# nichmorgan/better-search-rag-rust

Hardware: AMD Instinct MI355X
Metric: queries/sec + p50 latency, 768-d top-10 over N vectors @1/2/4/8 GPU (higher is better)
Workload: dtype f32; 1 GPU; configs[2]: 10M x 768 f32 corpus sharded over the N GPUs, 1000 batched queries, top-10; rows_total=10000000, rows_per_gpu_rank0=10000000, queries=1000, top_k=10, dim=768, parallelism=corpus sharded over 1 GPU(s) (interval_by_rank)

## Files before the change

better-search-rag-rust_amd/csrc/k_filter.hip:

```cpp
#include <cstdlib>
#include "bsr_device.hpp"
#include "kernels.hpp"

#include <hip/hip_ext.h>

#include <limits.h>
#include <math.h>

#include <algorithm>
#include <type_traits>
#include <utility>

namespace bsr {

typedef __attribute__((ext_vector_type(4))) int i32x4_t;
typedef __attribute__((ext_vector_type(16))) int i32x16_t;
typedef __attribute__((address_space(3))) void lds_void_t;

constexpr int kSlots = 4;
constexpr int kSliceB = 64;
constexpr int kWCap = 256;
constexpr int kThreads = 512;

__device__ __forceinline__ void wait_vm0() { asm volatile("s_waitcnt vmcnt(0)" ::: "memory"); }
// ... 307 lines not shown
        BSR_QS_N(1) BSR_QS_N(2) BSR_QS_N(3) BSR_QS_N(4) BSR_QS_N(5) BSR_QS_N(6) BSR_QS_N(7) BSR_QS_N(8)
        BSR_QS_N(9) BSR_QS_N(10) BSR_QS_N(11) BSR_QS_N(12) BSR_QS_N(13) BSR_QS_N(14) BSR_QS_N(15)
        default: qs_wait<0>(); break;
    }
#undef BSR_QS_N
}

#ifdef BSR_FILTER_STAMPS
__device__ __forceinline__ void qs_vm_n(int n) {
#define BSR_QS_V(N) \
    case N: asm volatile("s_waitcnt vmcnt(" #N ")" ::: "memory"); break;
    switch (n) {
        BSR_QS_V(1) BSR_QS_V(2) BSR_QS_V(3) BSR_QS_V(4) BSR_QS_V(5) BSR_QS_V(6) BSR_QS_V(7) BSR_QS_V(8)
        default: asm volatile("s_waitcnt vmcnt(0)" ::: "memory"); break;
    }
#undef BSR_QS_V
}
#endif
typedef __attribute__((ext_vector_type(4))) int i32x4v_t;

template <class F, int... I>
__device__ __forceinline__ void static_for(std::integer_sequence<int, I...>, F&& f) {
    (f(std::integral_constant<int, I>{}), ...);
}

constexpr int kSampleTilesPerWG = 8;

__device__ __forceinline__ uint32_t qs16_swz(uint32_t row) { return ((row >> 3) & 1u) * 2u; }

#ifdef BSR_FILTER_COUNTERS
__device__ unsigned long long g_filter_counters[8];
extern "C" int bsr_lab_filter_counters(unsigned long long* out, int reset) {
    hipError_t e = hipMemcpyFromSymbol(out, HIP_SYMBOL(g_filter_counters), sizeof(g_filter_counters));
    if (e == hipSuccess && reset) {
        static const unsigned long long z[8] = {};
        e = hipMemcpyToSymbol(HIP_SYMBOL(g_filter_counters), z, sizeof(z));
    }
    return (int)e;
}
__device__ unsigned long long g_filter_wg_stamps[4096 * 9];
__device__ uint32_t g_lab_xcd_xor;
extern "C" int bsr_lab_set_xcd_xor(uint32_t v) {
    return (int)hipMemcpyToSymbol(HIP_SYMBOL(g_lab_xcd_xor), &v, sizeof v);
}
__device__ unsigned int g_filter_wg_tiles[4096 * 2];
extern "C" int bsr_lab_filter_wg_tiles(unsigned int* out) {
    return (int)hipMemcpyFromSymbol(out, HIP_SYMBOL(g_filter_wg_tiles), sizeof(g_filter_wg_tiles));
}
extern "C" int bsr_lab_filter_wg_stamps(unsigned long long* out) {
    return (int)hipMemcpyFromSymbol(out, HIP_SYMBOL(g_filter_wg_stamps), sizeof(g_filter_wg_stamps));
}
#define BSR_FCNT(I_) ++fcnt[I_]
#else
#define BSR_FCNT(I_) \
    do {             \
    } while (0)
#endif
#ifdef BSR_FILTER_STAMPS
__device__ unsigned long long g_filter_stamps[8];
extern "C" int bsr_lab_filter_stamps(unsigned long long* out, int reset) {
    hipError_t e = hipMemcpyFromSymbol(out, HIP_SYMBOL(g_filter_stamps), sizeof(g_filter_stamps));
    if (e == hipSuccess && reset) {
        static const unsigned long long z[8] = {};
        e = hipMemcpyToSymbol(HIP_SYMBOL(g_filter_stamps), z, sizeof(z));
    }
    return (int)e;
}
#define BSR_FST(V_)                                                                     \
    do {                                                                                \
        __builtin_amdgcn_sched_barrier(0);                                              \
        asm volatile("s_memtime %0\n\ts_waitcnt lgkmcnt(0)" : "=s"(V_)::"memory");       \
        __builtin_amdgcn_sched_barrier(0);                                              \
    } while (0)
#endif
template <bool EMIT, int NK, bool GANGS = true>
__global__ __launch_bounds__(512, 1) void k_filter_qs16(GemmArgs p) {
    constexpr int GANG = GANGS ? 2 : 0;
    constexpr bool L2 = !GANGS, FW = GANGS;
    constexpr int S = 8, A = 6;
    constexpr int kWaitN = A - 4, kYoung = A - 4, kClaimUse = ((A - 4) % 2 == 0 ? A - 3 : A - 2) + 1;
    constexpr int BM = 128, BN = kFilterTile, NT = 512, SLOT = BM * kSliceB;
    constexpr int CAP = 10;
    static_assert(NK % 2 == 0 && NK >= 2 && NK <= 12, "even slice counts up to 768 bytes");
    constexpr int EM_BYTES = EMIT ? NT * 2 * CAP * 8 : 0;
    constexpr int SB_BYTES = EMIT ? 0 : kSampleTilesPerWG * 4 * BN * 4;
    __shared__ __attribute__((aligned(1024))) uint8_t lds[S * SLOT + EM_BYTES + SB_BYTES + 16];
    float* const sbuf = reinterpret_cast<float*>(lds + S * SLOT + EM_BYTES);
    uint32_t* const lds_ids = reinterpret_cast<uint32_t*>(lds + S * SLOT + EM_BYTES + SB_BYTES);
    const int tid = threadIdx.x, lane = tid & 63, w = tid >> 6;
    const uint32_t wu = __builtin_amdgcn_readfirstlane(tid >> 6);
    uint64_t* const lkeys = reinterpret_cast<uint64_t*>(lds + S * SLOT) + tid;
    uint32_t ecnt[2] = {0, 0};

    const uint32_t b = blockIdx.x, xcd = b & 7, slot = b >> 3;
    const uint32_t G = (gridDim.x >> 3) / p.n_qt;
    const uint32_t n_phys = (p.n_rows + BM - 1) / BM;
    const uint32_t n_rt = !p.s_tiles ? n_phys : EMIT ? n_phys - p.s_tiles : p.s_tiles;
    auto phys = [&](uint32_t lt) -> uint32_t {
        if (!p.s_tiles) return lt;
        return EMIT ? lt + lt / (kSampleTileEvery - 1) : lt * kSampleTileEvery + kSampleTilePhase;
    };
    const bool active = slot < G * p.n_qt;
    const uint32_t qt = active ? slot % p.n_qt : 0;
#ifdef BSR_FILTER_COUNTERS
    const uint32_t g0 = (xcd ^ g_lab_xcd_xor) * G + (active ? slot / p.n_qt : 0);
#else
    const uint32_t g0 = xcd * G + (active ? slot / p.n_qt : 0);
#endif
    const uint32_t RG = 8 * G;
    const uint32_t my_rt = (active && g0 < n_rt) ? (n_rt - 1 - g0) / RG + 1 : 0;
    const uint32_t J = my_rt * NK;
    constexpr uint32_t kEnd = 0xFFFFFFFFu;
    constexpr bool kStaticSched = NK > A;
    const bool dyn = EMIT && kStaticSched && p.tail != nullptr && active;
    const uint32_t n_st = dyn ? n_rt - n_rt / kTailDiv : n_rt;
    const uint32_t my_static = (active && g0 < n_st) ? (n_st - 1 - g0) / RG + 1 : 0;
    const uint32_t n_tail = n_rt - n_st, pool_sz = (n_tail + 7) / 8;
    uint32_t cpool = xcd, pools_tried = 1;
    auto pool_n = [&](uint32_t x) -> uint32_t {
        const uint32_t lo = x * pool_sz;
        return lo >= n_tail ? 0u : min(pool_sz, n_tail - lo);
    };
    auto claim_raw = [&]() -> uint32_t {
        uint32_t z;
        asm volatile("v_mov_b32 %0, 0" : "=v"(z));
        return atomicAdd(p.tail + cpool * p.n_qt + qt + z, 1u);
    };
    auto tail_id = [&](uint32_t v) -> uint32_t {
        for (;;) {
            if (v < pool_n(cpool)) return n_st + cpool * pool_sz + v;
            if (pools_tried == 8) return kEnd;
            ++pools_tried;
            cpool = (cpool + 1) & 7;
            v = atomicAdd(p.tail + cpool * p.n_qt + qt, 1u);
        }
    };
    auto claim = [&]() -> uint32_t { return tail_id(claim_raw()); };
    const bool gang = GANG && EMIT && kStaticSched && active && p.tail != nullptr && p.n_qt >= 2 && p.n_qt <= 4 &&
                      my_static >= kGangMinTiles;
    unsigned long long* const gprog =
        reinterpret_cast<unsigned long long*>(p.tail + 8 * kTailCounters) + (gang ? g0 : 0u);
    auto gang_raw = [&]() -> unsigned long long {
        uint32_t z;
        asm volatile("v_mov_b32 %0, 0" : "=v"(z));
        return atomicAdd(gprog + z, 1ull << (16 * qt));
    };
    auto gang_throttle = [&](unsigned long long old) {
        const uint32_t me = (uint32_t)(old >> (16 * qt)) & 0xFFFFu;
        int lag = 0;
        for (uint32_t j = 0; j < p.n_qt; ++j)
            if (j != qt) lag = max(lag, (int)(int16_t)(uint16_t)(me - ((uint32_t)(old >> (16 * j)) & 0xFFFFu)));
        for (int i = GANG; i < lag && i < GANG + 4; ++i) __builtin_amdgcn_s_sleep(32);
    };

    uint32_t qq[2];
    i32x4v_t fb[2][NK];
    float tau[2], sbq[2];
#pragma unroll
    for (int nb = 0; nb < 2; ++nb) {
        qq[nb] = qt * BN + w * 32 + nb * 16 + (lane & 15);
        const uint8_t* src = p.B + (uint64_t)qq[nb] * p.row_bytes + 16 * (lane >> 4);
#pragma unroll
        for (int kt = 0; kt < NK; ++kt) fb[nb][kt] = *reinterpret_cast<const i32x4v_t*>(src + 64 * kt);
        tau[nb] = EMIT ? p.tau[qq[nb]] : 0.0f;
        sbq[nb] = p.b_scale[qq[nb]];
    }
    auto flush_ring = [&](int nb) {
        const uint32_t nn = ecnt[nb];
        if (nn) {
            const uint32_t gp = atomicAdd(p.cnt + qq[nb], nn);
            for (uint32_t i = 0; i < nn; ++i)
                if (gp + i < p.cap) p.cand[(uint64_t)qq[nb] * p.cap + gp + i] = lkeys[(nb * CAP + i) * NT];
        }
        ecnt[nb] = 0;
        if constexpr (FW) __builtin_amdgcn_s_waitcnt(0x0F70);
    };

    const uint32_t lrow = w * 16 + (lane >> 2);
    const uint32_t lchunk = ((lane & 3) ^ qs16_swz(lrow)) * 16;
    auto tile_src_rt = [&](uint32_t lt, __amdgpu_buffer_rsrc_t& rs, uint32_t& off) {
        const uint32_t rt = phys(lt);
        rs = __builtin_amdgcn_make_buffer_rsrc((void*)(p.A + (uint64_t)rt * BM * p.a_stride), 0,
                                               BM * (uint32_t)p.a_stride, 0x00020000);
        const uint32_t r = (EMIT || rt * BM + lrow < p.n_rows) ? lrow : p.n_rows - 1 - rt * BM;
        off = r * (uint32_t)p.a_stride + lchunk;
    };
    auto tile_src = [&](uint32_t ti, __amdgpu_buffer_rsrc_t& rs, uint32_t& off) { tile_src_rt(g0 + ti * RG, rs, off); };
    constexpr bool kStatic = kStaticSched;
    __amdgpu_buffer_rsrc_t rs_cur, rs_nxt;
    uint32_t off_cur = 0, off_nxt = 0;
    auto dma_static = [&](uint32_t jj, int kt) {
        uint8_t* la = lds + (jj % S) * SLOT + wu * 1024;
        if (kt + A < NK)
            __builtin_amdgcn_raw_ptr_buffer_load_lds(rs_cur, (lds_void_t*)la, 16, off_cur, (kt + A) * kSliceB, 0, 0);
        else
            __builtin_amdgcn_raw_ptr_buffer_load_lds(rs_nxt, (lds_void_t*)la, 16, off_nxt, (kt + A - NK) * kSliceB, 0, 0);
    };
    uint32_t iss_ti = 0, iss_kt = 0, aoff_dma = 0;
    __amdgpu_buffer_rsrc_t rsrc_a;
    auto issue_dma = [&](uint32_t jj) {
        uint8_t* la = lds + (jj % S) * SLOT + wu * 1024;
        __builtin_amdgcn_raw_ptr_buffer_load_lds(rsrc_a, (lds_void_t*)la, 16, aoff_dma, iss_kt * kSliceB, 0, 0);
        if (++iss_kt == NK) {
            iss_kt = 0;
            ++iss_ti;
            if (iss_ti < my_rt) tile_src(iss_ti, rsrc_a, aoff_dma);
        }
    };
    const uint32_t aoff0 = (lane & 15) * kSliceB + (((lane >> 4) ^ qs16_swz(lane & 15)) * 16);
    i32x4v_t fa[4];
    auto read_frag = [&](uint32_t jj, int rb) {
        fa[rb & 3] = *reinterpret_cast<const i32x4v_t*>(lds + (jj % S) * SLOT + rb * 1024 + aoff0);
    };

    i32x4v_t acc[8][2];
    uint32_t cur_id = my_rt ? g0 : kEnd, nxt_id = my_rt > 1 ? g0 + RG : kEnd;
    if (dyn && my_static < 2) {
        if (tid == 0) {
            const uint32_t a0 = my_static ? g0 : claim();
            lds_ids[2] = a0;
            lds_ids[3] = a0 == kEnd ? kEnd : claim();
        }
        __syncthreads();
        cur_id = __builtin_amdgcn_readfirstlane(lds_ids[2]);
        nxt_id = __builtin_amdgcn_readfirstlane(lds_ids[3]);
    } else if (dyn) {
        cur_id = g0;
        nxt_id = g0 + RG;
    }
    const bool any_tile = cur_id != kEnd;
    const uint32_t pre = (dyn ? any_tile : J != 0) ? (uint32_t)A : 0u;
    if (any_tile) {
        tile_src_rt(cur_id, rsrc_a, aoff_dma);
        rs_cur = rsrc_a;
        off_cur = aoff_dma;
        tile_src_rt(nxt_id != kEnd ? nxt_id : cur_id, rs_nxt, off_nxt);
    }
    if (kStatic) {
        for (uint32_t jj = 0; jj < pre; ++jj) {
            uint8_t* la = lds + (jj % S) * SLOT + wu * 1024;
            __builtin_amdgcn_raw_ptr_buffer_load_lds(rs_cur, (lds_void_t*)la, 16, off_cur, jj * kSliceB, 0, 0);
        }
    } else {
        for (uint32_t jj = 0; jj < pre; ++jj) issue_dma(jj);
    }
    qs_barrier(pre >= 3 ? pre - 3 : 0);
    if (any_tile)
#pragma unroll
        for (int rb = 0; rb < 4; ++rb) read_frag(0, rb);

#ifdef BSR_FILTER_COUNTERS
    unsigned long long fcnt[5] = {0, 0, 0, 0, 0};
    if (EMIT && tid == 0 && blockIdx.x < 4096) g_filter_wg_stamps[blockIdx.x * 9] = __builtin_amdgcn_s_memrealtime();
#endif
#ifdef BSR_FILTER_STAMPS
    unsigned long long fst[8] = {0, 0, 0, 0, 0, 0, 0, 0}, st_a, st_b, st_loop0;
    BSR_FST(st_loop0);
#endif
// ... 52 lines not shown
                if (bar_slice ? rb == 6 : rb == 1) {
                    if (kStatic) dma_static(jj + A, kt);
                    else issue_dma(jj + A);
                }
                if (bar_slice && rb == 5 && (kStatic || jj + 1 < J)) {
#ifdef BSR_FILTER_STAMPS
                    if (EMIT) {
                        BSR_FST(st_a);
                        qs_vm_n(kWaitN + ((EMIT && kt <= kYoung) ? 1 + w0_req : 0));
                        BSR_FST(st_b);
                        fst[6] += st_b - st_a;
                        st_a = st_b;
                        asm volatile("s_barrier" ::: "memory");
                        BSR_FST(st_b);
                        fst[kt == 1 ? 3 : 4] += st_b - st_a;
                    } else
#endif
                    qs_wait_n(kWaitN + ((EMIT && kt <= kYoung) ? 1 + w0_req : 0));
                }
                __builtin_amdgcn_sched_barrier(0);
            }
        });
        const float sc[4] = {scv.x, scv.y, scv.z, scv.w};
        bool stored = false;
        if constexpr (!EMIT) {
            if (p.s_compact) {
                const bool part = p.s_tiles && rt * BM + BM > p.n_rows;
#pragma unroll
                for (int g = 0; g < 4; ++g)
#pragma unroll
                    for (int nb = 0; nb < 2; ++nb) {
                        i32x4v_t x = acc[2 * g][nb], y = acc[2 * g + 1][nb];
                        if (part) {
                            const uint32_t r0 = rt * BM + g * 32 + 4 * (lane >> 4);
#pragma unroll
                            for (int r = 0; r < 4; ++r) {
                                x[r] = r0 + r < p.n_rows ? x[r] : INT_MIN;
                                y[r] = r0 + 16 + r < p.n_rows ? y[r] : INT_MIN;
                            }
                        }
                        int m = max(max(max(x[0], x[1]), max(x[2], x[3])), max(max(y[0], y[1]), max(y[2], y[3])));
                        const auto p16 = __builtin_amdgcn_permlane16_swap(m, m, false, false);
                        m = max((int)p16[0], (int)p16[1]);
                        const auto p32 = __builtin_amdgcn_permlane32_swap(m, m, false, false);
                        m = max((int)p32[0], (int)p32[1]);
                        const float v = ((float)m * sc_blk[g]) * sbq[nb];
                        if (lane < 16) sbuf[((t % kSampleTilesPerWG) * 4 + g) * BN + (qq[nb] - qt * BN)] = v;
                    }
                if (t % kSampleTilesPerWG == kSampleTilesPerWG - 1 || t + 1 == my_rt) {
                    __syncthreads();
                    const uint32_t t0 = t - t % kSampleTilesPerWG, nt = t + 1 - t0;
                    for (uint32_t i = tid; i < nt * BN; i += NT) {
                        const uint32_t tt = i / BN, ql = i % BN;
                        const float4 v = make_float4(sbuf[(tt * 4 + 0) * BN + ql], sbuf[(tt * 4 + 1) * BN + ql],
                                                     sbuf[(tt * 4 + 2) * BN + ql], sbuf[(tt * 4 + 3) * BN + ql]);
                        *reinterpret_cast<float4*>(p.S + (uint64_t)(qt * BN + ql) * p.s_ld + (g0 + (t0 + tt) * RG) * 4) = v;
                    }
                    stored = true;
                }
            } else {
#pragma unroll
                for (int rb = 0; rb < 8; ++rb) {
                    const uint32_t rbase = rt * BM + rb * 16 + 4 * (lane >> 4);
#pragma unroll
                    for (int nb = 0; nb < 2; ++nb) {
                        const i32x4v_t& x = acc[rb][nb];
                        const float v0 = ((float)x[0] * sc_tile) * sbq[nb], v1 = ((float)x[1] * sc_tile) * sbq[nb];
                        const float v2 = ((float)x[2] * sc_tile) * sbq[nb], v3 = ((float)x[3] * sc_tile) * sbq[nb];
                        *reinterpret_cast<float4*>(p.S + (uint64_t)qq[nb] * p.s_ld + rbase) = make_float4(v0, v1, v2, v3);
                    }
                }
                stored = true;
            }
        } else {
            const float sc_hi = fmaxf(fmaxf(sc[0], sc[1]), fmaxf(sc[2], sc[3]));
            const float sc_lo = fminf(fminf(sc[0], sc[1]), fminf(sc[2], sc[3]));
            bool any = false;
            BSR_FCNT(0);
#ifdef BSR_FILTER_STAMPS
            BSR_FST(st_a);
            fst[7] += 1;
#endif
            int mrb[2];
#pragma unroll
            for (int nb = 0; nb < 2; ++nb) {
                int m = acc[0][nb][0];
#pragma unroll
                for (int rb = 0; rb < 8; ++rb)
#pragma unroll
                    for (int r = 0; r < 4; ++r) m = (rb | r) ? max(m, acc[rb][nb][r]) : m;
                mrb[nb] = m;
                any |= ((float)m * (m >= 0 ? sc_hi : sc_lo)) * sbq[nb] >= tau[nb];
            }
            const bool l2 = __ballot(any) != 0;
#ifdef BSR_FILTER_STAMPS
            BSR_FST(st_b);
            fst[0] += st_b - st_a;
            st_a = st_b;
#endif
            if (l2) {
                BSR_FCNT(1);
#pragma unroll
                for (int nb = 0; nb < 2; ++nb) {
                    if (!__ballot(((float)mrb[nb] * (mrb[nb] >= 0 ? sc_hi : sc_lo)) * sbq[nb] >= tau[nb])) continue;
                    BSR_FCNT(2);
                    uint32_t pm = 0;
                    bool pass_rb[8];
#pragma unroll
                    for (int rb = 0; rb < 8; ++rb) {
                        const i32x4v_t& x = acc[rb][nb];
                        const int bm = max(max(x[0], x[1]), max(x[2], x[3]));
                        if constexpr (L2) pass_rb[rb] = ((float)bm * sc[rb >> 1]) * sbq[nb] >= tau[nb];
                        else pm |= (((float)bm * sc[rb >> 1]) * sbq[nb] >= tau[nb]) ? 1u << rb : 0u;
                    }
#pragma unroll
                    for (int rb = 0; rb < 8; ++rb) {
                        if (!__ballot(L2 ? pass_rb[rb] : ((pm >> rb) & 1u))) continue;
                        BSR_FCNT(3);
                        if (__ballot(ecnt[nb] > (uint32_t)(CAP - 4))) {
                            flush_ring(nb);
                            stored = true;
                        }
                        const i32x4v_t& x = acc[rb][nb];
                        const float scr = sc[rb >> 1];
#pragma unroll
                        for (int r = 0; r < 4; ++r) {
                            const float v = ((float)x[r] * scr) * sbq[nb];
                            const uint32_t row = rt * BM + rb * 16 + 4 * (lane >> 4) + r;
                            lkeys[(nb * CAP + ecnt[nb]) * NT] = score_key(v, row);
                            ecnt[nb] += (v >= tau[nb] && row < p.n_rows) ? 1u : 0u;
                        }
                    }
                }
#ifdef BSR_FILTER_STAMPS
                BSR_FST(st_b);
                fst[1] += st_b - st_a;
                fst[2] += 1;
#endif
            }
        }
        if (stored) wait_vm0();
        cur_id = nxt_id;
        nxt_id = req ? __builtin_amdgcn_readfirstlane(lds_ids[t & 1]) : n2;
    }
    wait_vm0();
#ifdef BSR_FILTER_STAMPS
    if (EMIT) {
        BSR_FST(st_b);
        fst[5] = st_b - st_loop0;
        if (lane == 0)
            for (int i = 0; i < 8; ++i) atomicAdd(&g_filter_stamps[i], fst[i]);
    }
#endif
    if constexpr (EMIT) {
        flush_ring(0);
        flush_ring(1);
#ifdef BSR_FILTER_COUNTERS
        if (lane == 0) {
            for (int i = 0; i < 4; ++i) atomicAdd(&g_filter_counters[i], fcnt[i]);
            if (blockIdx.x < 4096) g_filter_wg_stamps[blockIdx.x * 9 + 1 + w] = __builtin_amdgcn_s_memrealtime();
            if (blockIdx.x < 4096 && w == 0) {
                g_filter_wg_tiles[blockIdx.x * 2] = (unsigned int)fcnt[4];
                g_filter_wg_tiles[blockIdx.x * 2 + 1] = my_static;
            }
        }
#endif
    }
}


__global__ __launch_bounds__(256) void k_sample_fixup(GemmArgs p) {
    constexpr int NKM = 12, U = 4;
    const uint32_t q = blockIdx.x;
    const float tq = p.tau[q];
    if (!(tq < INFINITY)) return;
    const int tid = threadIdx.x, lane = tid & 63;
    const uint32_t w0 = __builtin_amdgcn_readfirstlane(tid >> 6) * 64;
    const uint32_t c = lane & 3, rr = lane >> 2;
    const int nk = p.row_bytes / kSliceB;
    const float sbq = p.b_scale[q];
    i32x4_t fb[NKM];
#pragma unroll
    for (int s = 0; s < NKM; ++s)
        fb[s] = s < nk ? *reinterpret_cast<const i32x4_t*>(p.B + (uint64_t)q * p.row_bytes + s * kSliceB + c * 16)
                       : i32x4_t{0, 0, 0, 0};
    auto block = [&](uint32_t j) {
        const uint32_t r0 = ((j >> 2) * kSampleTileEvery + kSampleTilePhase) * 128 + (j & 3) * 32;
        const float sc = p.a_scale[r0 / kQuantBlock];
        i32x4_t fa[2][NKM];
#pragma unroll
        for (int h = 0; h < 2; ++h) {
            const uint8_t* a = p.A + (uint64_t)(r0 + 16 * h + rr) * p.a_stride + c * 16;
#pragma unroll
            for (int s = 0; s < NKM; ++s)
                if (s < nk) fa[h][s] = *reinterpret_cast<const i32x4_t*>(a + s * kSliceB);
        }
#pragma unroll
        for (int h = 0; h < 2; ++h) {
            int acc = 0;
#pragma unroll
            for (int s = 0; s < NKM; ++s)
                if (s < nk)
#pragma unroll
                    for (int e = 0; e < 4; ++e) acc = __builtin_amdgcn_sdot4(fa[h][s][e], fb[s][e], acc, false);
            acc += (int)xor_lane32<1>((uint32_t)acc);
            acc += (int)xor_lane32<2>((uint32_t)acc);
            const float v = ((float)acc * sc) * sbq;
            const uint32_t row = r0 + 16 * h + rr;
            const bool pass = c == 0 && v >= tq && row < p.n_rows;
            const uint64_t mk = __ballot(pass);
            if (mk) {
                uint32_t gp = 0;
                if (lane == 0) gp = atomicAdd(p.cnt + q, (uint32_t)__builtin_popcountll(mk));
                gp = __builtin_amdgcn_readfirstlane(gp);
                const uint32_t pos = gp + (uint32_t)__builtin_popcountll(mk & ((1ull << lane) - 1ull));
                if (pass && pos < p.cap) p.cand[(uint64_t)q * p.cap + pos] = score_key(v, row);
            }
        }
    };
    const float* srow = p.S + (uint64_t)q * p.s_ld;
    for (uint32_t base = 0; base < p.s_vals; base += U * 256) {
        float sv[U];
#pragma unroll
        for (int u = 0; u < U; ++u) {
            const uint32_t j = base + u * 256 + tid;
            sv[u] = j < p.s_vals ? srow[j] : -INFINITY;
        }
#pragma unroll
        for (int u = 0; u < U; ++u) {
            const uint32_t j = base + u * 256 + tid;
            uint64_t m = __ballot(j < p.s_vals && sv[u] >= tq);
            while (m) {
                const uint32_t b = (uint32_t)__builtin_ctzll(m);
                m &= m - 1;
                block(base + u * 256 + w0 + b);
            }
        }
    }
}
// ... 660 lines not shown

#define BSR_KLAUNCH(K, G, B, S, A) hipLaunchKernelGGL(K, G, B, 0, S, A)

static uint32_t skinny_grid(uint32_t n_rows) {
    const uint32_t groups = (n_rows + 31) / 32, wgs = (groups + 3) / 4;
    return wgs < 768 ? (wgs ? wgs : 1) : 768;
}
static uint32_t skinny2_grid(uint32_t n_rows) {
    const uint32_t units = (n_rows + 15) / 16;
    return std::min<uint32_t>(512, std::max<uint32_t>(1, (units + 3) / 4));
}
uint32_t skinny_top_lists(uint32_t n_rows) { return skinny2_grid(n_rows); }
bool skinny_glds_on() {
    const char* v = getenv("BSR_SKINNY_GLDS");
    return !(v && v[0] == '0');
}
template <int MODE>
static void launch_skinny(const GemmArgs& a, hipStream_t s) {
    const uint32_t nk = a.row_bytes / kSliceB;
    if constexpr (MODE != kSkSample) {
        if (nk == 12 && skinny_glds_on()) {
            BSR_KLAUNCH((k_filter_skinny_glds<MODE, 12>), dim3(skinny2_grid(a.n_rows)), dim3(128), s, a);
            return;
        }
    }
    const dim3 g(nk <= 16 ? skinny2_grid(a.n_rows) : skinny_grid(a.n_rows)), b(256);
    if (nk <= 4) BSR_KLAUNCH((k_filter_skinny2<MODE, 4>), g, b, s, a);
    else if (nk <= 8) BSR_KLAUNCH((k_filter_skinny2<MODE, 8>), g, b, s, a);
    else if (nk <= 12) BSR_KLAUNCH((k_filter_skinny2<MODE, 12>), g, b, s, a);
    else if (nk <= 16) BSR_KLAUNCH((k_filter_skinny2<MODE, 16>), g, b, s, a);
    else if constexpr (MODE != kSkTop) BSR_KLAUNCH(k_filter_skinny<MODE == kSkEmit>, g, b, s, a);
}
hipError_t launch_filter_skinny_sample(const GemmArgs& a, hipStream_t s) {
    launch_skinny<kSkSample>(a, s);
    return hipGetLastError();
}
hipError_t launch_filter_skinny_emit(const GemmArgs& a, hipStream_t s) {
    launch_skinny<kSkEmit>(a, s);
    return hipGetLastError();
}
hipError_t launch_filter_skinny_top(const GemmArgs& a, hipStream_t s) {
    if (a.row_bytes / kSliceB > 16) return hipErrorInvalidValue;
    launch_skinny<kSkTop>(a, s);
    return hipGetLastError();
}

static bool gang_possible(const GemmArgs& a, uint32_t grid) {
    if (!a.tail || a.n_qt < 2 || a.n_qt > 4) return false;
    const uint32_t G = (grid / 8) / a.n_qt, RG = 8 * G;
    const uint32_t n_rt = (a.n_rows + 127) / 128 - a.s_tiles, n_st = n_rt - n_rt / kTailDiv;
    return RG && n_st && (n_st - 1) / RG + 1 >= kGangMinTiles;
}

template <bool EMIT>
static void launch_filter(const GemmArgs& a, hipStream_t s) {
    const uint32_t nk = a.row_bytes / kSliceB, grid = filter_grid(a.n_qt);
    if (nk % 2 == 0 && nk <= 12) {
        const dim3 g(grid), b(512);
        if constexpr (EMIT) {
            if (nk == 12 && !gang_possible(a, grid)) {
                BSR_KLAUNCH((k_filter_qs16<true, 12, false>), g, b, s, a);
                return;
            }
        }
        switch (nk) {
            case 2: BSR_KLAUNCH((k_filter_qs16<EMIT, 2>), g, b, s, a); return;
            case 4: BSR_KLAUNCH((k_filter_qs16<EMIT, 4>), g, b, s, a); return;
            case 6: BSR_KLAUNCH((k_filter_qs16<EMIT, 6>), g, b, s, a); return;
            case 8: BSR_KLAUNCH((k_filter_qs16<EMIT, 8>), g, b, s, a); return;
            case 10: BSR_KLAUNCH((k_filter_qs16<EMIT, 10>), g, b, s, a); return;
            default: BSR_KLAUNCH((k_filter_qs16<EMIT, 12>), g, b, s, a); return;
        }
    }
    BSR_KLAUNCH((k_filter<EMIT>), dim3(grid), dim3(kThreads), s, a);
}
hipError_t launch_filter_sample(const GemmArgs& a, hipStream_t s) {
    launch_filter<false>(a, s);
    return hipGetLastError();
}
hipError_t launch_filter_emit(const GemmArgs& a, hipStream_t s) {
    launch_filter<true>(a, s);
    return hipGetLastError();
}
hipError_t launch_sample_fixup(const GemmArgs& a, hipStream_t s) {
    const uint32_t nk = a.row_bytes / kSliceB;
    if (!a.s_tiles || !a.n_q || nk < 1 || nk > 12 || a.row_bytes % kSliceB) return hipErrorInvalidValue;
    hipLaunchKernelGGL(k_sample_fixup, dim3(a.n_q), dim3(256), 0, s, a);
    return hipGetLastError();
}
template <bool PQ>
static void launch_select_tau_pq(const float* S, uint32_t s_ld, uint32_t n_s, uint32_t nq, uint32_t qpad,
                                 const uint32_t* qflags, uint32_t ks, float* tau, uint32_t* cnt, uint32_t* status,
                                 hipStream_t s, uint64_t* smax, const uint32_t* ks_q) {
    static const int m_on = [] {
        const char* v = getenv("BSR_SELECT_TAU_M");
        return v && v[0] == '0' ? 0 : v && v[0] == '2' ? 2 : 1;
    }();
    if (m_on && ks <= kWave && (qpad <= 16 || m_on == 2) && n_s > 32 * kWave && n_s <= 16 * 16 * kWave)
        hipLaunchKernelGGL((k_select_tau_m<16, PQ>), dim3(qpad), dim3(1024), 0, s, S, s_ld, n_s, nq, qpad, qflags, ks,
                           tau, cnt, status, smax, ks_q);
    else if (ks <= kWave && n_s <= 32 * kWave && qpad % 4 == 0)
        hipLaunchKernelGGL((k_select_tau_w<32, PQ>), dim3(qpad / 4), dim3(256), 0, s, S, s_ld, n_s, nq, qpad, qflags,
                           ks, tau, cnt, status, smax, ks_q);
    else if (ks > kWave)
        hipLaunchKernelGGL((k_select_tau<2, PQ>), dim3(qpad), dim3(256), 0, s, S, s_ld, n_s, nq, qpad, qflags, ks, tau,
                           cnt, status, smax, ks_q);
    else
        hipLaunchKernelGGL((k_select_tau<1, PQ>), dim3(qpad), dim3(256), 0, s, S, s_ld, n_s, nq, qpad, qflags, ks, tau,
                           cnt, status, smax, ks_q);
}
hipError_t launch_select_tau(const float* S, uint32_t s_ld, uint32_t n_s, uint32_t nq, uint32_t qpad,
                             const uint32_t* qflags, uint32_t ks, float* tau, uint32_t* cnt, uint32_t* status,
                             hipStream_t s, uint64_t* smax, const uint32_t* ks_q) {
    if (ks > 2 * kWave || (ks_q && smax)) return hipErrorInvalidValue;
    if (ks_q) launch_select_tau_pq<true>(S, s_ld, n_s, nq, qpad, qflags, ks, tau, cnt, status, s, smax, ks_q);
    else launch_select_tau_pq<false>(S, s_ld, n_s, nq, qpad, qflags, ks, tau, cnt, status, s, smax, ks_q);
    return hipGetLastError();
}
hipError_t launch_global_tau(const uint64_t* g, uint32_t P, uint32_t qpad, uint32_t nq, uint32_t ks,
                             const uint32_t* qflags, float* tau, hipStream_t s) {
    if (ks > 2 * kWave || P == 0) return hipErrorInvalidValue;
    if (ks > kWave)
        hipLaunchKernelGGL(k_global_tau<2>, dim3(qpad / 4), dim3(256), 0, s, g, P, qpad, nq, ks, qflags, tau);
    else
        hipLaunchKernelGGL(k_global_tau<1>, dim3(qpad / 4), dim3(256), 0, s, g, P, qpad, nq, ks, qflags, tau);
    return hipGetLastError();
}
hipError_t launch_select_cand(const uint64_t* cand, const uint32_t* cnt, uint32_t cap, uint32_t nq,
                              const float* tau, uint32_t kp, uint32_t* cand_rows, uint32_t* ncand,
                              float* tau_excl, hipStream_t s) {
    const uint32_t e = (kp + 1 + 63) / 64;
#define BSR_SELECT(E)                                                                                   \
    hipLaunchKernelGGL(k_select_cand<E>, dim3(nq), dim3(64), 0, s, cand, cnt, cap, nq, tau, kp, cand_rows, \
                       ncand, tau_excl)
    switch (e) {
        case 1: BSR_SELECT(1); break;
        case 2: BSR_SELECT(2); break;
        case 3: BSR_SELECT(3); break;
        case 4: BSR_SELECT(4); break;
        case 5: BSR_SELECT(5); break;
        case 6: BSR_SELECT(6); break;
        case 7: BSR_SELECT(7); break;
        case 8: BSR_SELECT(8); break;
        case 9: BSR_SELECT(9); break;
        case 10: BSR_SELECT(10); break;
        default: return hipErrorInvalidValue;
    }
#undef BSR_SELECT
    return hipGetLastError();
}

}
```

better-search-rag-rust_amd/csrc/kernels.hpp:

```cpp
#pragma once

#include <hip/hip_runtime.h>
#include <stdint.h>

namespace bsr {

constexpr uint32_t kLdAlign = 64;
constexpr uint32_t kRowPad = 256;
constexpr uint32_t kScanQF = 8;
constexpr uint32_t kSampleStride = 32;
constexpr uint32_t kQuantBlock = 32;
constexpr uint32_t kSampleScaleRows = 128;
constexpr uint32_t kFilterTile = 256;

constexpr uint32_t kRowNonFinite = 1u;
constexpr uint32_t kRowNormOvf = 2u;
constexpr uint32_t kRowNormRange = 4u;

constexpr uint32_t kQueryNonFinite = 1u;
constexpr uint32_t kQueryNoApprox = 2u;

enum StatusWord : uint32_t { kStFail = 0, kStEmitted = 1, kStQueryFlags = 2, kStFail2 = 3, kStWords = 4 };

hipError_t launch_synth_uniform(float* out, uint64_t row0, uint64_t n_rows, uint32_t dim,
// ... 32 lines not shown

constexpr uint32_t kMaskBlockWords = 256;
static inline uint32_t mask_blocks(uint64_t n) {
    const uint64_t words = (n + 63) / 64, b = (words + kMaskBlockWords - 1) / kMaskBlockWords;
    return (uint32_t)(b < 1 ? 1 : b);
}
hipError_t launch_mask_list_count(const uint64_t* allow, uint64_t n, uint32_t* blk, hipStream_t s);
hipError_t launch_mask_list_scatter(const uint64_t* allow, uint64_t n, const uint32_t* blk, uint32_t n_list,
                                    uint32_t* list, hipStream_t s);
hipError_t launch_mask_cut(uint64_t* cand, uint32_t* cnt, uint32_t cap, uint32_t nq, const uint64_t* allow,
                           uint64_t n, uint32_t* raw, uint32_t* items, hipStream_t s);

hipError_t launch_mask_groups_count(const uint64_t* allow, uint64_t words, uint32_t n_masks, uint64_t n,
                                    const uint64_t* dead, const uint32_t* query_mask, uint32_t nq, uint32_t* blk,
                                    uint32_t* out, hipStream_t s);
struct MaskListDesc { uint64_t off; uint32_t mask, n_list; };
hipError_t launch_mask_groups_scatter(const uint64_t* allow, uint64_t words, uint64_t n, const uint64_t* dead,
                                      const uint32_t* blk, const MaskListDesc* d, uint32_t n_lists, uint32_t* list,
                                      hipStream_t s);
hipError_t launch_mask_cut_groups(uint64_t* cand, uint32_t* cnt, uint32_t cap, uint32_t nq, const uint64_t* allow,
                                  uint64_t words, const uint32_t* query_mask, const uint64_t* dead, uint64_t n,
                                  uint32_t* raw, uint32_t* items, hipStream_t s);
struct ScanGroupDesc { uint64_t off; uint32_t n_list, nq; };

hipError_t launch_dead_check(const uint64_t* ids, uint64_t n_ids, uint64_t lo, uint64_t n, uint32_t* bad,
                             hipStream_t s);
hipError_t launch_dead_apply(const uint64_t* ids, uint64_t n_ids, uint64_t lo, uint64_t n, uint64_t* dead,
                             uint32_t* newly, hipStream_t s);
hipError_t launch_dead_zero_fop(const uint64_t* dead, uint64_t n, const uint32_t* dead_blk, uint32_t row_bytes,
                                uint8_t* fop, uint8_t* fop_s, const float* rows, uint32_t dim, const float* scales_s,
                                hipStream_t s);
hipError_t launch_dead_andnot(const uint64_t* allow, const uint64_t* dead, uint64_t n, uint64_t* out, hipStream_t s);

enum UpdCount : uint32_t { kUpdBadId = 0, kUpdDupId = 1, kUpdNonFinite = 2, kUpdSampleRows = 3, kUpdCounts = 4 };
hipError_t launch_upd_check(const uint64_t* ids, uint64_t n_ids, uint64_t lo, uint64_t n, const void* src,
                            uint32_t dim, bool bf16, uint64_t* touched, uint64_t* blocks, uint64_t* groups,
                            uint64_t* cnt, hipStream_t s);
hipError_t launch_upd_scatter(const uint64_t* ids, uint64_t n_ids, uint64_t lo, const void* src, uint32_t dim,
                              uint32_t ld, bool bf16, float* rows, hipStream_t s);
hipError_t launch_upd_row_norms(const float* rows, const uint64_t* ids, uint64_t n_ids, uint64_t lo, uint32_t dim,
                                uint32_t ld, float* na, uint32_t* flags, hipStream_t s);
hipError_t launch_upd_rows_to_i8(const float* rows, uint64_t n, uint32_t dim, uint32_t ld, int8_t* out, float* scales,
                                 uint32_t* ea_max, const uint32_t* list, const uint32_t* count, uint32_t cap,
                                 hipStream_t s);
hipError_t launch_upd_rows_to_i8_sample(const float* rows, uint64_t n, uint32_t dim, uint32_t ld, int8_t* out,
                                        float* scales, const uint32_t* list, const uint32_t* count, uint32_t cap,
                                        hipStream_t s);

hipError_t launch_compact_gather(const float* rows, const uint32_t* list, uint64_t cnt, uint32_t ld, float* out,
                                 hipStream_t s);
hipError_t launch_compact_ids(const uint32_t* list, uint64_t cnt, uint64_t lo, uint64_t* out, uint32_t* first,
                              hipStream_t s);

struct GemmArgs {
    const uint8_t* A;
    uint64_t a_stride;
    uint32_t n_rows;
    uint32_t a_scale_rows;
    const uint8_t* B;
    uint32_t row_bytes;
    uint32_t n_rt, n_qt;
    const float* a_scale;
    const float* b_scale;
    float* S;
    uint32_t s_ld;
    uint32_t s_compact;
    const float* tau;
    uint64_t* cand;
    uint32_t* cnt;
    uint32_t cap;
    uint32_t* tail;
    uint32_t* status;
    uint32_t n_q;
    uint32_t top_layout;
    uint32_t s_tiles, s_vals;
};
constexpr uint32_t kSampleTileEvery = 32;
constexpr uint32_t kSampleTilePhase = 31;
static inline uint32_t sample_tiles_for(uint64_t n) { return (uint32_t)(((n + 127) / 128) / kSampleTileEvery); }
constexpr uint32_t kTailDiv = 8;
constexpr uint32_t kTailCounters = 64;
constexpr uint32_t kGangWords = 2 * 256;
constexpr uint32_t kGangMinTiles = 600;
hipError_t launch_filter_sample(const GemmArgs& a, hipStream_t s);
hipError_t launch_filter_emit(const GemmArgs& a, hipStream_t s);
hipError_t launch_sample_fixup(const GemmArgs& a, hipStream_t s);
constexpr uint32_t kSkinnyMaxQ = 16;
hipError_t launch_filter_skinny_sample(const GemmArgs& a, hipStream_t s);
hipError_t launch_filter_skinny_emit(const GemmArgs& a, hipStream_t s);
hipError_t launch_filter_skinny_top(const GemmArgs& a, hipStream_t s);
uint32_t skinny_top_lists(uint32_t n_rows);
bool skinny_glds_on();
constexpr uint64_t kSkinnyTopMinRows = 2u << 20;

hipError_t launch_select_tau(const float* S, uint32_t s_ld, uint32_t n_s, uint32_t nq,
                             uint32_t qpad, const uint32_t* qflags, uint32_t ks, float* tau,
                             uint32_t* cnt, uint32_t* status, hipStream_t s, uint64_t* smax = nullptr,
                             const uint32_t* ks_q = nullptr);
hipError_t launch_global_tau(const uint64_t* g, uint32_t P, uint32_t qpad, uint32_t nq, uint32_t ks,
                             const uint32_t* qflags, float* tau, hipStream_t s);
hipError_t launch_select_cand(const uint64_t* cand, const uint32_t* cnt, uint32_t cap,
                              uint32_t nq, const float* tau, uint32_t kp, uint32_t* cand_rows,
                              uint32_t* ncand, float* tau_excl, hipStream_t s);

struct RescoreArgs {
    const float* rows;
    uint32_t ld, dim;
    const float* na;
    const float* qf32;
    const float* nb;
    uint32_t n_items;
    const uint32_t* n_items_dev;
    const uint32_t* qlist;
    const uint32_t* cand_rows;
    const uint32_t* ncand;
    uint32_t kp;
    const float* tau_excl;
    const uint64_t* cand_keys;
    const uint32_t* cnt;
    uint32_t cap;
    const float* tau0;
    uint32_t sel;
    uint32_t top_w;
    const uint32_t* qflags;
    float* top_tau;
    uint32_t* top_cnt;
    uint32_t k;
    const float* ebound;
    uint64_t* out_keys;
    uint32_t* fail_cnt;
    uint32_t* fail_list;
    uint64_t* res_idx;
    float* res_dist;
    uint32_t* res_cnt;
    uint64_t offset, n_rows;
    const uint64_t* dead;
    uint64_t* hres_idx;
    float* hres_dist;
    uint32_t* hres_cnt;
    uint32_t* next_status;
    const uint32_t* emit_cnt;
    uint32_t* cur_status;
    uint32_t n_queries;
    float* excl_out;
    uint32_t* merge_words;
    const uint8_t* pub_src;
    uint8_t* pub_dst;
    size_t pub_bytes;
    uint32_t* pub_flag;
    uint32_t* pub_ticket;
    uint32_t solo;
};
constexpr uint32_t kTicketLeaves = 8, kTicketStride = 16, kTicketWords = (kTicketLeaves + 1) * kTicketStride;
constexpr uint32_t kRescoreAllGrid = 128;
constexpr uint32_t kFusedSelectCap = 1024;
hipError_t launch_rescore(const RescoreArgs& a, hipStream_t s);
bool rescore_kp_enabled();
constexpr uint32_t kTopKeysPerLane = 32;
hipError_t launch_scan_exact(const float* rows, uint32_t ld, uint32_t dim, uint64_t n,
                             const float* na, const float* qf32, const int32_t* qids,
                             uint32_t nqf, const float* nb, uint32_t k, uint32_t grid,
                             uint64_t* part, hipStream_t s);
hipError_t launch_merge_parts(const uint64_t* part, uint32_t grid, const int32_t* qids,
                              uint32_t nqf, uint32_t k, uint64_t* out_keys, hipStream_t s);
hipError_t launch_scan_list(const float* rows, uint32_t ld, uint32_t dim, const uint32_t* list,
                            uint32_t n_list, const float* na, const float* qf32, const int32_t* qids,
                            uint32_t nqf, uint32_t groups, const float* nb, uint32_t k, uint32_t grid,
                            uint64_t* part, hipStream_t s);
// ... 52 lines not shown
```

Measured before the change: 174,300 queries/s.

## Buffer filter survivors in a per-wave LDS queue and flush one record per lane

For the 768-byte gang emit filter, a lane whose coarse bound passes no longer runs the per-row-block ballot cascade. It now copies its whole 8x4 accumulator block, with a header and row scales, into a per-wave LDS queue of 48 records. When the queue fills, each lane takes one record, re-checks the 32 scores against that query's tau (read from a shared LDS table) and writes survivors to the candidate list with a single atomic per record. The aim is to remove the divergence and serialised ballots of the old per-lane ring, at the cost of more LDS (queues plus table) and extra LDS traffic per passing lane. A new gang emit launcher is also added.

```diff
diff --git a/better-search-rag-rust_amd/csrc/k_filter.hip b/better-search-rag-rust_amd/csrc/k_filter.hip
--- a/better-search-rag-rust_amd/csrc/k_filter.hip
+++ b/better-search-rag-rust_amd/csrc/k_filter.hip
@@ -413,7 +413,11 @@
     constexpr int BM = 128, BN = kFilterTile, NT = 512, SLOT = BM * kSliceB;
     constexpr int CAP = 10;
     static_assert(NK % 2 == 0 && NK >= 2 && NK <= 12, "even slice counts up to 768 bytes");
-    constexpr int EM_BYTES = EMIT ? NT * 2 * CAP * 8 : 0;
+    constexpr bool QUEUE = GANGS && EMIT && NK == 12;
+    constexpr int QD = kEmitQueueDepth, REC_B = 144, HDR_B = 32, QW_BYTES = QD * (REC_B + HDR_B);
+    static_assert(QD >= 1 && QD <= kWave, "the flush takes one record per lane");
+    constexpr int EM_BYTES = QUEUE ? 8 * QW_BYTES + 2 * BN * 4 : EMIT ? NT * 2 * CAP * 8 : 0;
+    static_assert(S * SLOT + EM_BYTES + 16 <= 160 * 1024, "the ring, the queues and the table fit one CU's LDS");
     constexpr int SB_BYTES = EMIT ? 0 : kSampleTilesPerWG * 4 * BN * 4;
     __shared__ __attribute__((aligned(1024))) uint8_t lds[S * SLOT + EM_BYTES + SB_BYTES + 16];
     float* const sbuf = reinterpret_cast<float*>(lds + S * SLOT + EM_BYTES);
@@ -505,6 +509,56 @@
         }
         ecnt[nb] = 0;
         if constexpr (FW) __builtin_amdgcn_s_waitcnt(0x0F70);
+    };
+    uint8_t* const qrec = lds + S * SLOT + wu * QW_BYTES;
+    uint8_t* const qhdr = qrec + QD * REC_B;
+    float* const tab_tau = reinterpret_cast<float*>(lds + S * SLOT + 8 * QW_BYTES);
+    float* const tab_bs = tab_tau + BN;
+    uint32_t nrec = 0;
+    if constexpr (QUEUE) {
+        if (lane < 16) {
+#pragma unroll
+            for (int nb = 0; nb < 2; ++nb) {
+                tab_tau[wu * 32 + nb * 16 + lane] = tau[nb];
+                tab_bs[wu * 32 + nb * 16 + lane] = sbq[nb];
+            }
+        }
+    }
+    auto flush_queue = [&]() {
+        if ((uint32_t)lane < nrec) {
+            const uint8_t* hd = qhdr + lane * HDR_B;
+            const uint2 h = *reinterpret_cast<const uint2*>(hd);
+            const float4 s4 = *reinterpret_cast<const float4*>(hd + 16);
+            const uint32_t ql = wu * 32 + (h.y >> 6) * 16 + (h.y & 15u);
+            const float tq = tab_tau[ql], sq = tab_bs[ql];
+            const uint32_t row0 = h.x * BM + 4 * ((h.y >> 4) & 3u);
+            const uint8_t* rr = qrec + lane * REC_B;
+            uint32_t pm = 0;
+#pragma unroll 1
+            for (int rb = 0; rb < 8; ++rb) {
+                const i32x4v_t x = *reinterpret_cast<const i32x4v_t*>(rr + rb * 16);
+                const float scr = (rb >> 1) == 0 ? s4.x : (rb >> 1) == 1 ? s4.y : (rb >> 1) == 2 ? s4.z : s4.w;
+#pragma unroll
+                for (int r = 0; r < 4; ++r) {
+                    const float v = ((float)x[r] * scr) * sq;
+                    pm |= (v >= tq && row0 + rb * 16 + r < p.n_rows) ? 1u << (rb * 4 + r) : 0u;
+                }
+            }
+            if (pm) {
+                const uint32_t q = qt * BN + ql;
+                uint32_t gp = atomicAdd(p.cnt + q, (uint32_t)__builtin_popcount(pm));
+                __builtin_amdgcn_s_waitcnt(0x0F70);
+                for (; pm; pm &= pm - 1, ++gp) {
+                    const uint32_t i = (uint32_t)__builtin_ctz(pm);
+                    const int I = *reinterpret_cast<const int*>(rr + i * 4);
+                    const float scr = (i >> 3) == 0 ? s4.x : (i >> 3) == 1 ? s4.y : (i >> 3) == 2 ? s4.z : s4.w;
+                    const float v = ((float)I * scr) * sq;
+                    if (gp < p.cap) p.cand[(uint64_t)q * p.cap + gp] = score_key(v, row0 + (i >> 2) * 16 + (i & 3));
+                }
+            }
+        }
+        nrec = 0;
+        __builtin_amdgcn_s_waitcnt(0x0F70);
     };
 
     const uint32_t lrow = w * 16 + (lane >> 2);
@@ -723,6 +777,7 @@
             fst[7] += 1;
 #endif
             int mrb[2];
+            bool l1p[2];
 #pragma unroll
             for (int nb = 0; nb < 2; ++nb) {
                 int m = acc[0][nb][0];
@@ -731,7 +786,8 @@
 #pragma unroll
                     for (int r = 0; r < 4; ++r) m = (rb | r) ? max(m, acc[rb][nb][r]) : m;
                 mrb[nb] = m;
-                any |= ((float)m * (m >= 0 ? sc_hi : sc_lo)) * sbq[nb] >= tau[nb];
+                l1p[nb] = ((float)m * (m >= 0 ? sc_hi : sc_lo)) * sbq[nb] >= tau[nb];
+                any |= l1p[nb];
             }
             const bool l2 = __ballot(any) != 0;
 #ifdef BSR_FILTER_STAMPS
@@ -741,35 +797,66 @@
 #endif
             if (l2) {
                 BSR_FCNT(1);
-#pragma unroll
-                for (int nb = 0; nb < 2; ++nb) {
-                    if (!__ballot(((float)mrb[nb] * (mrb[nb] >= 0 ? sc_hi : sc_lo)) * sbq[nb] >= tau[nb])) continue;
-                    BSR_FCNT(2);
-                    uint32_t pm = 0;
-                    bool pass_rb[8];
-#pragma unroll
-                    for (int rb = 0; rb < 8; ++rb) {
-                        const i32x4v_t& x = acc[rb][nb];
-                        const int bm = max(max(x[0], x[1]), max(x[2], x[3]));
-                        if constexpr (L2) pass_rb[rb] = ((float)bm * sc[rb >> 1]) * sbq[nb] >= tau[nb];
-                        else pm |= (((float)bm * sc[rb >> 1]) * sbq[nb] >= tau[nb]) ? 1u << rb : 0u;
+                if constexpr (QUEUE) {
+                    const uint64_t lbit = 1ull << lane;
+#pragma unroll
+                    for (int nb = 0; nb < 2; ++nb) {
+                        uint64_t bal = __ballot(l1p[nb]);
+                        while (bal) {
+                            if (nrec == (uint32_t)QD) {
+                                flush_queue();
+                                stored = true;
+                            }
+                            const uint32_t rank =
+                                __builtin_amdgcn_mbcnt_hi((uint32_t)(bal >> 32), __builtin_amdgcn_mbcnt_lo((uint32_t)bal, 0u));
+                            const bool mine = (bal & lbit) && rank < (uint32_t)QD - nrec;
+                            if (mine) {
+                                const uint32_t sl = nrec + rank;
+#pragma unroll
+                                for (int rb = 0; rb < 8; ++rb)
+                                    *reinterpret_cast<i32x4v_t*>(qrec + sl * REC_B + rb * 16) = acc[rb][nb];
+                                const i32x4v_t hv = {(int)rt, nb << 6 | lane, 0, 0};
+                                const i32x4v_t sv = {(int)__float_as_uint(scv.x), (int)__float_as_uint(scv.y),
+                                                     (int)__float_as_uint(scv.z), (int)__float_as_uint(scv.w)};
+                                *reinterpret_cast<i32x4v_t*>(qhdr + sl * HDR_B) = hv;
+                                *reinterpret_cast<i32x4v_t*>(qhdr + sl * HDR_B + 16) = sv;
+                            }
+                            const uint64_t took = __ballot(mine);
+                            nrec += (uint32_t)__builtin_popcountll(took);
+                            bal &= ~took;
+                        }
                     }
-#pragma unroll
-                    for (int rb = 0; rb < 8; ++rb) {
-                        if (!__ballot(L2 ? pass_rb[rb] : ((pm >> rb) & 1u))) continue;
-                        BSR_FCNT(3);
-                        if (__ballot(ecnt[nb] > (uint32_t)(CAP - 4))) {
-                            flush_ring(nb);
-                            stored = true;
+                } else {
+#pragma unroll
+                    for (int nb = 0; nb < 2; ++nb) {
+                        if (!__ballot(((float)mrb[nb] * (mrb[nb] >= 0 ? sc_hi : sc_lo)) * sbq[nb] >= tau[nb])) continue;
+                        BSR_FCNT(2);
+                        uint32_t pm = 0;
+                        bool pass_rb[8];
+#pragma unroll
+                        for (int rb = 0; rb < 8; ++rb) {
+                            const i32x4v_t& x = acc[rb][nb];
+                            const int bm = max(max(x[0], x[1]), max(x[2], x[3]));
+                            if constexpr (L2) pass_rb[rb] = ((float)bm * sc[rb >> 1]) * sbq[nb] >= tau[nb];
+                            else pm |= (((float)bm * sc[rb >> 1]) * sbq[nb] >= tau[nb]) ? 1u << rb : 0u;
                         }
-                        const i32x4v_t& x = acc[rb][nb];
-                        const float scr = sc[rb >> 1];
-#pragma unroll
-                        for (int r = 0; r < 4; ++r) {
-                            const float v = ((float)x[r] * scr) * sbq[nb];
-                            const uint32_t row = rt * BM + rb * 16 + 4 * (lane >> 4) + r;
-                            lkeys[(nb * CAP + ecnt[nb]) * NT] = score_key(v, row);
-                            ecnt[nb] += (v >= tau[nb] && row < p.n_rows) ? 1u : 0u;
+#pragma unroll
+                        for (int rb = 0; rb < 8; ++rb) {
+                            if (!__ballot(L2 ? pass_rb[rb] : ((pm >> rb) & 1u))) continue;
+                            BSR_FCNT(3);
+                            if (__ballot(ecnt[nb] > (uint32_t)(CAP - 4))) {
+                                flush_ring(nb);
+                                stored = true;
+                            }
+                            const i32x4v_t& x = acc[rb][nb];
+                            const float scr = sc[rb >> 1];
+#pragma unroll
+                            for (int r = 0; r < 4; ++r) {
+                                const float v = ((float)x[r] * scr) * sbq[nb];
+                                const uint32_t row = rt * BM + rb * 16 + 4 * (lane >> 4) + r;
+                                lkeys[(nb * CAP + ecnt[nb]) * NT] = score_key(v, row);
+                                ecnt[nb] += (v >= tau[nb] && row < p.n_rows) ? 1u : 0u;
+                            }
                         }
                     }
                 }
@@ -794,8 +881,12 @@
     }
 #endif
     if constexpr (EMIT) {
-        flush_ring(0);
-        flush_ring(1);
+        if constexpr (QUEUE) {
+            flush_queue();
+        } else {
+            flush_ring(0);
+            flush_ring(1);
+        }
 #ifdef BSR_FILTER_COUNTERS
         if (lane == 0) {
             for (int i = 0; i < 4; ++i) atomicAdd(&g_filter_counters[i], fcnt[i]);
@@ -1622,6 +1713,11 @@
     launch_filter<true>(a, s);
     return hipGetLastError();
 }
+hipError_t launch_filter_emit_gang(const GemmArgs& a, hipStream_t s) {
+    if (a.row_bytes != 12 * kSliceB) return hipErrorInvalidValue;
+    BSR_KLAUNCH((k_filter_qs16<true, 12, true>), dim3(filter_grid(a.n_qt)), dim3(512), s, a);
+    return hipGetLastError();
+}
 hipError_t launch_sample_fixup(const GemmArgs& a, hipStream_t s) {
     const uint32_t nk = a.row_bytes / kSliceB;
     if (!a.s_tiles || !a.n_q || nk < 1 || nk > 12 || a.row_bytes % kSliceB) return hipErrorInvalidValue;
diff --git a/better-search-rag-rust_amd/csrc/kernels.hpp b/better-search-rag-rust_amd/csrc/kernels.hpp
--- a/better-search-rag-rust_amd/csrc/kernels.hpp
+++ b/better-search-rag-rust_amd/csrc/kernels.hpp
@@ -138,8 +138,10 @@
 constexpr uint32_t kTailCounters = 64;
 constexpr uint32_t kGangWords = 2 * 256;
 constexpr uint32_t kGangMinTiles = 600;
+constexpr int kEmitQueueDepth = 48;
 hipError_t launch_filter_sample(const GemmArgs& a, hipStream_t s);
 hipError_t launch_filter_emit(const GemmArgs& a, hipStream_t s);
+hipError_t launch_filter_emit_gang(const GemmArgs& a, hipStream_t s);
 hipError_t launch_sample_fixup(const GemmArgs& a, hipStream_t s);
 constexpr uint32_t kSkinnyMaxQ = 16;
 hipError_t launch_filter_skinny_sample(const GemmArgs& a, hipStream_t s);
```

Measured after the change: 177,500 queries/s (median of 6 runs). +1.8%, better.
